# timgluz/teeline

Hardware: AMD Instinct MI355X
Metric: 2-opt candidate swaps evaluated/sec + final tour cost, TSPLIB EUC_2D n=10000 (higher is better)
Workload: dtype f32

## Files before the change

teeline_amd/csrc/two_opt_ref.hip:

```cpp
#include "tl_kernels.h"
#include "two_opt_common.h"

#include <type_traits>

#pragma clang fp contract(off)

namespace tl {

namespace {

constexpr uint32_t kNoKey = 0xFFFFFFFFu;
#if defined(TL_PROFILE2) || defined(TL_PROFILE3)
constexpr bool kProbeOwnsStats = true;
#else
constexpr bool kProbeOwnsStats = false;
#endif
#ifndef TL_RMAX
#define TL_RMAX 63
#endif
#ifndef TL_DENSE_ROWS
#define TL_DENSE_ROWS 8.0f
#endif
constexpr int kRMax = TL_RMAX;
constexpr uint32_t kQCap = 32;
constexpr uint32_t kPendMax = 64;
constexpr int kFlushSlots = 15;
constexpr int kFlushSlotsFx = 20;
constexpr int kMaxGroups = 4;


struct Ctl {
    uint2 kr[4];
    uint32_t desc[4];
    unsigned long long cnt[6];
    unsigned long long clk0, rt0;
    uint32_t bad_init;
    uint32_t nlong;
    uint32_t late_cur;
    uint32_t pad_[1];
    uint32_t pend[64];
};
constexpr size_t kCtlBytes = 384;
static_assert(sizeof(Ctl) <= kCtlBytes, "Ctl block");

constexpr size_t kXyBytes = 8, kFxLoBytes = 4, kFxHiBytes = 1, kPermBytes = 2, kNlPosBytes = 2;
constexpr size_t kTboxBytes = kMaxGroups * 64 * 16, kTmsqBytes = kMaxGroups * 64 * 4, kQueuesBytes = 32 * kQCap * 4;
constexpr size_t kNlLongBytes = (size_t)kNlLongCap * 16, kNlSurvBytes = 16 * 64 * 2;
static_assert(kQueuesBytes >= TL_TWO_OPT_NT * 4, "the hit lists double as the cost-sum scratch");

template <int CTRL>
__device__ __forceinline__ uint32_t dpp_shr0(uint32_t v)
{
    return (uint32_t)__builtin_amdgcn_update_dpp(0, (int)v, CTRL, 0xf, 0xf, true);
}
__device__ __forceinline__ uint32_t readlane_u(uint32_t v, uint32_t l) { return (uint32_t)__builtin_amdgcn_readlane((int)v, (int)l); }

template <int NT, int SLOTS, typename PT>
__device__ __forceinline__ uint32_t flush_deferred(const PT &P, uint16_t *perm, uint32_t g, uint32_t lo, uint32_t k, int lane, int wave)
{
    using Raw = decltype(pt_raw(P, 0u));
    const bool have = (uint32_t)lane < k;
    const uint32_t ghi = readlane_u(g, k - 1u);
    const uint32_t wfirst = lo + ((uint32_t)wave << 6);
    Raw val[SLOTS];
    uint32_t pk[SLOTS];
    if (wfirst <= ghi) {
        uint32_t gprev = dpp_shr0<0x111>(g);
        gprev = lane == 16 ? readlane_u(g, 15) : gprev;
        gprev = lane == 32 ? readlane_u(g, 31) : gprev;
        gprev = lane == 48 ? readlane_u(g, 47) : gprev;
        gprev = lane == 0 ? lo - 1u : gprev;
        const uint32_t start = gprev + 1u;
        const uint32_t len = have ? g - gprev : 0u;
        uint32_t pre = len;
        pre += dpp_shr0<0x112>(pre);
        pre += dpp_shr0<0x114>(pre);
        pre += dpp_shr0<0x118>(pre);
        if (k > 16u) {
            const uint32_t e0 = readlane_u(pre, 14), o0 = readlane_u(pre, 15);
            const uint32_t e1 = e0 + readlane_u(pre, 30), o1 = o0 + readlane_u(pre, 31);
            const uint32_t e2 = e1 + readlane_u(pre, 46), o2 = o1 + readlane_u(pre, 47);
            const bool odd = (lane & 1) != 0;
            uint32_t off = 0u;
            off = lane >= 16 ? (odd ? o0 : e0) : off;
            off = lane >= 32 ? (odd ? o1 : e1) : off;
            off = lane >= 48 ? (odd ? o2 : e2) : off;
            pre += off;
        }
        const uint32_t t_rev = readlane_u(pre, k - 1u);
        const bool isrev = ((k - 1u - (uint32_t)lane) & 1u) == 0u;
        const uint32_t base = lo + (isrev ? t_rev - pre : t_rev + pre - len);
        const uint32_t cst = isrev ? base + g : base - start;
#pragma unroll
        for (int q = 0; q < SLOTS; ++q) {
            const uint32_t w0 = wfirst + (uint32_t)(q * NT);
            if (w0 > ghi) break;
            const uint32_t p = w0 + (uint32_t)lane;
            const uint32_t w1 = (w0 + 63u < ghi) ? w0 + 63u : ghi;
            uint32_t m = (uint32_t)__builtin_popcountll(__builtin_amdgcn_ballot_w64(g < w0));
            const uint32_t mhi = (uint32_t)__builtin_popcountll(__builtin_amdgcn_ballot_w64(g < w1));
            const uint32_t c0 = readlane_u(cst, m);
            uint32_t dst = ((k - 1u - m) & 1u) == 0u ? c0 - p : c0 + p;
            for (++m; m <= mhi; ++m) {
                const uint32_t sm = readlane_u(start, m), cm = readlane_u(cst, m);
                const bool rv = ((k - 1u - m) & 1u) == 0u;
                dst = p >= sm ? (rv ? cm - p : cm + p) : dst;
            }
            if (p <= ghi) {
                val[q] = pt_raw(P, p);
                pk[q] = (uint32_t)perm[p] | (dst << 16);
            }
        }
    }
    TL_SYNC();
    if (wfirst <= ghi) {
#pragma unroll
        for (int q = 0; q < SLOTS; ++q) {
            const uint32_t w0 = wfirst + (uint32_t)(q * NT);
            if (w0 > ghi) break;
            if (w0 + (uint32_t)lane <= ghi) {
                const uint32_t dst = pk[q] >> 16;
                pt_put(P, dst, val[q]);
                perm[dst] = (uint16_t)pk[q];
            }
        }
    }
    TL_SYNC();
    return have ? g - (lo - 1u) : 0u;
}

template <int NT, typename PT>
__device__ __forceinline__ void reverse_segment(const PT &P, uint16_t *perm, uint32_t lo, uint32_t hi, int tid, uint16_t *pos = nullptr)
{
    const uint32_t half = (hi - lo + 1u) >> 1;
    for (uint32_t t = (uint32_t)tid; t < half; t += 2 * NT) {
        const uint32_t t2 = t + NT;
        const bool two = t2 < half;
        const auto x = pt_raw(P, lo + t), y = pt_raw(P, hi - t);
        const uint16_t u = perm[lo + t], v = perm[hi - t];
        uint16_t u2 = u, v2 = v;
        auto x2 = x, y2 = y;
        if (two) {
            x2 = pt_raw(P, lo + t2);
            y2 = pt_raw(P, hi - t2);
            u2 = perm[lo + t2];
            v2 = perm[hi - t2];
        }
        pt_put(P, lo + t, y);
        pt_put(P, hi - t, x);
        perm[lo + t] = v;
        perm[hi - t] = u;
        if (pos) {
            pos[v] = (uint16_t)(lo + t);
            pos[u] = (uint16_t)(hi - t);
        }
        if (two) {
            pt_put(P, lo + t2, y2);
            pt_put(P, hi - t2, x2);
            perm[lo + t2] = v2;
            perm[hi - t2] = u2;
            if (pos) {
                pos[v2] = (uint16_t)(lo + t2);
                pos[u2] = (uint16_t)(hi - t2);
            }
        }
    }
}

struct Cursor {
    uint32_t i0, j0;
    uint32_t np;
    uint32_t slot, par;
    uint32_t dirty_lo, dirty_hi;
    bool pruned;
};
struct Acct {
    uint64_t moves, reversed, rev_lane;
    float gap_est, since;
    bool improved;
    uint32_t *log;
    uint32_t log_cap, log_n;
};

__device__ __forceinline__ uint32_t block_rows(const Cursor &c, uint32_t nrows)
{
    return c.pruned ? ((uint32_t)kRMax < nrows - c.i0 ? (uint32_t)kRMax : nrows - c.i0) : 1u;
}

__device__ __forceinline__ void log_word(Acct &a, int lane, uint32_t w)
{
    if (a.log) {
        if (lane == 0 && a.log_n < a.log_cap) a.log[a.log_n] = w;
        a.log_n += 1u;
    }
}

template <bool CONTROL, int NT, int SLOTS, typename PT>
__device__ __forceinline__ void flush_pending(Cursor &c, Acct &a, const PT &P, uint16_t *perm, Ctl *ctl, int lane, int wave, bool sync_first)
{
    if (sync_first) TL_SYNC();
    uint32_t g = ctl->pend[lane];
    g = (uint32_t)lane < c.np ? g : 0xFFFFFFFFu;
    const uint32_t ghi = readlane_u(g, c.np - 1u);
    const uint32_t r = flush_deferred<NT, SLOTS>(P, perm, g, c.i0 + 1u, c.np, lane, wave);
    if (CONTROL) {
        a.rev_lane += r;
        if (a.log) {
            const uint32_t at = a.log_n + (uint32_t)lane;
            if ((uint32_t)lane < c.np && at < a.log_cap) a.log[at] = (c.i0 << 16) | g;
            a.log_n += c.np;
        }
    }
    const uint32_t t0 = c.i0 >> 6, t1 = ghi >> 6;
    c.dirty_lo = t0 < c.dirty_lo ? t0 : c.dirty_lo;
    c.dirty_hi = t1 > c.dirty_hi ? t1 : c.dirty_hi;
    c.np = 0;
}

template <bool CONTROL, int NT, int SLOTS, bool FOLD, typename PT>
__device__ __forceinline__ bool step_boundary(Cursor &c, Acct &a, const PT &P, uint16_t *perm, Ctl *ctl, const uint32_t *queues, uint32_t n, uint32_t nrows,
                                              uint32_t R, int lane, int wave, int tid, uint32_t my_hits, float &bx, float &by, bool &reload, float *tmsq)
{
    const uint2 kr = ctl->kr[c.slot];
    const uint32_t key = (uint32_t)__builtin_amdgcn_readfirstlane((int)kr.x);
    const uint32_t req = (uint32_t)__builtin_amdgcn_readfirstlane((int)kr.y);
    const float rowlen = (float)(n - 2u - c.i0);
    reload = false;
    if (!c.pruned) {
        bool flush = false, sync_first = false, next_row = false;
        if (key == kNoKey) {
            if (CONTROL) a.since += rowlen;
            flush = c.np != 0u;
            next_row = true;
        } else {
            const uint4 hv = *reinterpret_cast<const uint4 *>(queues + ((key & 0xFFFFu) * 2u + c.par) * kQCap);
            const uint32_t nh = (uint32_t)__builtin_amdgcn_readfirstlane((int)hv.x);
            const uint32_t resume = (uint32_t)__builtin_amdgcn_readfirstlane((int)hv.y);
            if (!CONTROL && (key & 0xFFFFu) == (uint32_t)wave && (uint32_t)lane < nh) ctl->pend[c.np + (uint32_t)lane] = my_hits;
            if (CONTROL) {
                a.moves += nh;
                a.since += (float)((key >> 16) - c.j0);
                a.gap_est = 0.5f * (a.gap_est + a.since);
                a.since = 0.0f;
                if (nh > 1u) a.gap_est = fminf(a.gap_est, 0.5f * a.gap_est + 16.0f);
                a.improved = true;
            }
            c.np += nh;
            c.j0 = resume;
            next_row = c.j0 > n - 2u;
            flush = next_row || c.np + kMaxChainHits > kPendMax;
            sync_first = true;
            if (!flush) {
                bx = __builtin_bit_cast(float, __builtin_amdgcn_readfirstlane((int)hv.z));
                by = __builtin_bit_cast(float, __builtin_amdgcn_readfirstlane((int)hv.w));
            }
        }
        if (flush) flush_pending<CONTROL, NT, SLOTS>(c, a, P, perm, ctl, lane, wave, sync_first);
        if (next_row) {
            c.i0 += 1u;
            c.j0 = c.i0 + 2u;
        }
        reload = flush || next_row;
    } else if (key == kNoKey) {
        if (CONTROL) a.since += (float)R * rowlen;
        c.i0 += R;
        c.j0 = c.i0 + 2u;
    } else {
        const uint32_t is = key >> 16, js = key & 0xFFFFu;
        const uint32_t t0 = is >> 6, t1 = js >> 6;
        const bool fold = FOLD && t0 == t1;
        if (fold && tid == 0) {
            const float m = fmaxf(sqdist(pt_get(P, is), pt_get(P, js)), sqdist(pt_get(P, is + 1u), pt_get(P, js + 1u)));
            if (m > tmsq[t0]) tmsq[t0] = m;
        }
        reverse_segment<NT>(P, perm, is + 1u, js, tid);
        TL_SYNC();
        if (CONTROL) {
            log_word(a, lane, key);
            a.since += (float)(is - c.i0) * rowlen;
            a.moves += 1u;
            a.reversed += (uint64_t)(js - is);
            a.since += (req != 0u && is > c.i0) ? (float)(js - (is + 2u)) : (float)(js - c.j0);
            a.gap_est = 0.5f * (a.gap_est + a.since);
            a.since = 0.0f;
            a.improved = true;
        }
        if (!fold) {
            c.dirty_lo = t0 < c.dirty_lo ? t0 : c.dirty_lo;
            c.dirty_hi = t1 > c.dirty_hi ? t1 : c.dirty_hi;
        }
        c.i0 = is;
        c.j0 = js + 1u;
        if (c.j0 > n - 2u) {
            c.i0 += 1u;
            c.j0 = c.i0 + 2u;
        }
    }
    c.slot = c.slot == 2u ? 0u : c.slot + 1u;
    c.par ^= 1u;
    return c.i0 >= nrows || req != 0u;
}


struct NlLds {
    uint16_t *pos;
    uint4 *longe;
    uint16_t *surv;
};

template <typename PT>
__device__ __forceinline__ uint32_t nl_r2_bits(const PT &P, uint32_t k, uint32_t n)
{
    const float2 pk = pt_get(P, k);
    uint32_t r2 = 0u;
    if (k >= 1u) r2 = __builtin_bit_cast(uint32_t, sqdist(pt_get(P, k - 1u), pk));
    if (k + 1u < n) {
        const uint32_t s = __builtin_bit_cast(uint32_t, sqdist(pk, pt_get(P, k + 1u)));
        r2 = s > r2 ? s : r2;
// ... 225 lines not shown
                        if (q + 1u < (uint32_t)kLateRowsPerWave) recw = load_rec(cida, cidb, r + 1u);
                        else recw = load_rec(ida, idb, r0n);
                    }
                    const float rax = readlane_f(rp.x, r), ray = readlane_f(rp.y, r);
                    const float rbx = readlane_f(rq.x, r), rby = readlane_f(rq.y, r);
                    const float rsqab = readlane_f(rowsq, r);
                    const uint32_t jmin = (i == i0) ? j0 : (i + 2u);
                    tc.prow += 1u;
                    uint32_t col = 0xFFFFFFFFu;
                    bool listed = false;
                    if (nl_rows) {
                        const uint32_t w = cur & 0xFFFFu;
                        const bool bad = lane == 0 ? !((__builtin_bit_cast(uint32_t, rsqab) >> 16) < w) : (lane == 2 && w != 0u);
                        if (!__builtin_amdgcn_ballot_w64(bad)) {
                            listed = true;
                            uint32_t u = lane >= kNlSurv0 ? surv8 : w;
                            const bool valid = lane >= kNlRecA0 && u != 0xFFFFu;
                            u = valid ? u : 0u;
                            const uint32_t pu = L.pos[u];
                            uint32_t j = lane < kNlRecB0 ? pu : pu - 1u;
                            j = valid ? j : 0xFFFFFFFFu;
                            col = nl_pass(P, n, j, jmin, rax, ray, rbx, rby, rsqab, lane, tc);
                            if (ns > (uint32_t)kNlSurvSlots) {
                                const uint32_t q2 = (uint32_t)kNlSurvSlots + (uint32_t)lane;
                                const bool v2 = q2 < ns;
                                const uint32_t u2 = v2 ? sv[q2 < 64u ? q2 : 0u] : 0u;
                                const uint32_t p2 = L.pos[u2];
                                const uint32_t c2 = nl_pass(P, n, v2 ? p2 - 1u : 0xFFFFFFFFu, jmin, rax, ray, rbx, rby, rsqab, lane, tc);
                                col = c2 < col ? c2 : col;
                            }
                        }
                    }
                    if (!listed) {
                        float4 box[kMaxGroups];
                        float msq[kMaxGroups];
#pragma unroll
                        for (int gI = 0; gI < kMaxGroups; ++gI) {
                            if (gI < G) {
                                box[gI] = tbox[((uint32_t)gI << 6) + (uint32_t)lane];
                                msq[gI] = tmsq[((uint32_t)gI << 6) + (uint32_t)lane];
                            }
                        }
                        col = row_tiles<true>(P, n, G, box, msq, jmin, rax, ray, rbx, rby, rsqab, lane, tc);
                    }
                    TL_LSTAMP(2);
#ifdef TL_PROFILE_LATE
                    lq[3] += 1;
#endif
                    if (col == 0xFFFFFFFFu) continue;
                    if (lane == 0) lds_min_u32_fenced(keyslot, (i << 16) | col);
                    stop = true;
                    break;
                }
                g = gn;
            }
            TL_LSTAMP(5);
        }
#ifdef TL_PROFILE_LATE
        const uint64_t tb2 = __builtin_amdgcn_s_memtime();
#endif
        TL_SYNC();
#ifdef TL_PROFILE_LATE
        lq[4] += __builtin_amdgcn_s_memtime() - tb2;
#endif
        const uint32_t key = (uint32_t)__builtin_amdgcn_readfirstlane((int)ctl->kr[slot].x);
        if (key == kNoKey) {
            i0 += R;
            j0 = i0 + 2u;
        } else {
            const uint32_t is = key >> 16, js = key & 0xFFFFu;
            const uint32_t t0 = is >> 6, t1 = js >> 6;
            if (t0 == t1 && tid == 0) {
                const float m = fmaxf(sqdist(pt_get(P, is), pt_get(P, js)), sqdist(pt_get(P, is + 1u), pt_get(P, js + 1u)));
                if (m > tmsq[t0]) tmsq[t0] = m;
            }
            reverse_segment<NT>(P, perm, is + 1u, js, tid, L.pos);
            TL_SYNC();
            if (control) {
                log_word(acct, lane, key);
                acct.moves += 1u;
                acct.reversed += (uint64_t)(js - is);
            }
            improved = true;
            if (t0 != t1) {
                dirty_lo = t0 < dirty_lo ? t0 : dirty_lo;
                dirty_hi = t1 > dirty_hi ? t1 : dirty_hi;
            }
            fix = true;
            fi = is;
            fj = js;
            i0 = is;
            j0 = js + 1u;
            if (j0 > n - 2u) {
                i0 += 1u;
                j0 = i0 + 2u;
            }
        }
        slot = slot_next;
    }
#ifdef TL_PROFILE_LATE
    if (d == 0 && lane == 0 && (wave == 1 || wave == 9))
        printf("late phase, wave %d: chunk set-up %lu, prefilter %lu, rows %lu cycles in %lu rows (%lu per row), B2 wait %lu, other %lu\n", wave, lq[0], lq[1], lq[2], lq[3],
               lq[2] / (lq[3] ? lq[3] : 1), lq[4], lq[5]);
#endif
    (void)d;
}

}

template <int NT, bool PRUNE, bool COUNT, bool FX, bool NL = false>
__global__ __launch_bounds__(NT, 4) void k_two_opt_ref_lds(TwoOptBatchArgs A)
{
    static_assert(!NL || (PRUNE && !FX), "late phase: the float2 forms with pruning");
    constexpr int kSlots = FX ? kFlushSlotsFx : kFlushSlots;
    extern __shared__ __attribute__((aligned(16))) unsigned char smem[];
    constexpr int NW = NT / 64;
    static_assert(NW == 16 || NW == 8 || NW == 4, "16 waves; 8 or 4 for two or four descents per CU");
    const uint32_t n = A.n, npad = A.n_pad;
    const uint32_t ntile = npad >> 6;
    const int G = (int)((ntile + 63u) >> 6);
    using PT = typename std::conditional<FX, PtsFx, float2 *>::type;
    PT P;
    uint16_t *perm;
    unsigned char *tailp;
    if constexpr (FX) {
        P.lo = reinterpret_cast<uint32_t *>(smem);
        P.hi = reinterpret_cast<uint8_t *>(smem + (size_t)npad * kFxLoBytes);
        P.inv = A.fx_inv;
        perm = reinterpret_cast<uint16_t *>(smem + (size_t)npad * (kFxLoBytes + kFxHiBytes));
        tailp = smem + (size_t)npad * (kFxLoBytes + kFxHiBytes + kPermBytes);
    } else {
        P = reinterpret_cast<float2 *>(smem);
        perm = reinterpret_cast<uint16_t *>(smem + (size_t)npad * kXyBytes);
        tailp = smem + (size_t)npad * (kXyBytes + kPermBytes);
    }
    float4 *tbox = reinterpret_cast<float4 *>(tailp);
    float *tmsq = reinterpret_cast<float *>(tailp + kTboxBytes);
    Ctl *ctl = reinterpret_cast<Ctl *>(tailp + kTboxBytes + kTmsqBytes);
    uint32_t *queues = reinterpret_cast<uint32_t *>(reinterpret_cast<unsigned char *>(ctl) + kCtlBytes);
    float *scratch = reinterpret_cast<float *>(queues);
    NlLds L{nullptr, nullptr, nullptr};
    if constexpr (NL) {
        unsigned char *nlp = reinterpret_cast<unsigned char *>(queues) + kQueuesBytes;
        L.pos = reinterpret_cast<uint16_t *>(nlp);
        L.longe = reinterpret_cast<uint4 *>(nlp + (size_t)npad * kNlPosBytes);
        L.surv = reinterpret_cast<uint16_t *>(nlp + (size_t)npad * kNlPosBytes + kNlLongBytes);
    }

    const int tid = threadIdx.x, lane = tid & 63;
    const int wave = __builtin_amdgcn_readfirstlane(tid >> 6);
    const uint32_t d = blockIdx.x;
    const float2 *__restrict__ xy = A.xy;

    if (A.init_mode == TL_INIT_ARRAY) {
        const uint32_t *__restrict__ src = A.init + (size_t)d * n;
        if (tid == 0) ctl->bad_init = 0u;
        TL_SYNC();
        bool bad = false;
        for (uint32_t k = tid; k < n; k += NT) {
            const uint32_t v = src[k];
            bad |= v >= n;
            perm[k] = (uint16_t)v;
        }
        if (bad) ctl->bad_init = 1u;
        TL_SYNC();
        if (ctl->bad_init) {
            if (tid == 0) {
                A.out_cost[d] = __builtin_nanf("");
                uint64_t *st = A.out_stats + (size_t)d * TL_STATS_STRIDE;
                for (int q = 0; q < TL_STATS_STRIDE; ++q) st[q] = 0;
                st[3] = 2;
            }
            return;
        }
    } else {
        for (uint32_t k = tid; k < n; k += NT) perm[k] = (uint16_t)k;
    }
    if (A.init_mode == TL_INIT_SEEDED) {
        uint16_t *draws = reinterpret_cast<uint16_t *>(smem);
        const uint64_t s = A.seed + (uint64_t)(A.first + d);
        for (uint32_t i = 1 + tid; i < n; i += NT) {
            const uint64_t kth = (uint64_t)(n - 1 - i);
            draws[i] = (uint16_t)(splitmix64_at(s, kth) % ((uint64_t)i + 1));
        }
        TL_SYNC();
        if (tid == 0) {
            for (uint32_t i = n - 1; i >= 1; --i) {
                const uint32_t j = draws[i];
                const uint16_t t = perm[i];
                perm[i] = perm[j];
                perm[j] = t;
            }
        }
    }
    if (tid < 4) ctl->kr[tid] = make_uint2(kNoKey, 0u);
    if (tid < 6) ctl->cnt[tid] = 0ull;
    if (tid == 0) {
        ctl->nlong = 0u;
        ctl->clk0 = __builtin_amdgcn_s_memtime();
        ctl->rt0 = __builtin_amdgcn_s_memrealtime();
    }
    for (uint32_t k = tid; k < (uint32_t)kMaxGroups * 64u; k += NT) {
        const float inf = __builtin_inff();
        tbox[k] = make_float4(inf, inf, -inf, -inf);
        tmsq[k] = -1.0f;
    }
    TL_SYNC();
    if constexpr (FX) {
        for (uint32_t k = tid; k < npad; k += NT) {
            const uint2 g = (k < n) ? A.fx_xy[perm[k]] : make_uint2(0u, 0u);
            pt_put(P, k, PtsFx::Raw{g.x, g.y});
        }
    } else {
        for (uint32_t k = tid; k < npad; k += NT) P[k] = (k < n) ? xy[perm[k]] : make_float2(0.f, 0.f);
    }
    TL_SYNC();
    for (uint32_t t = (uint32_t)wave; t < ntile; t += NW) build_tile_meta(P, n, t, lane, tbox, tmsq);
    TL_SYNC();

    const uint32_t nrows = n - 3;
    const uint32_t last_tile = n >= 2 ? (n - 2u) >> 6 : 0u;
    uint32_t sweeps = 1, step = 0, status = 0;
    uint64_t moves = 0, reversed = 0;
    uint64_t rev_lane = 0;
    typename std::conditional<COUNT, TileCounts, NoCounts>::type tc;

    enum : uint32_t { OP_GO = 0u, OP_LATE = 1u, OP_EXIT = 2u };
    bool go_late = false;
    uint32_t n_late_steps = 0;
    uint64_t late_clk = 0;
    constexpr int NWK = NW - 1;
    constexpr uint32_t kLead = kDenseLead < (uint32_t)NWK ? kDenseLead : (uint32_t)NWK;
    if (n >= 4 && wave == 0) {
        Cursor c{0u, 2u, 0u, 0u, 0u, 0xFFFFFFFFu, 0u, false};
        Acct acct{0ull, 0ull, 0ull, 0.0f, 0.0f, false, A.move_log ? A.move_log + (size_t)d * A.log_cap : nullptr, A.log_cap, 0u};
        bool need_desc = true;
        uint32_t n_desc = 0, n_pruned_steps = 0;
        uint64_t sweep_moves0 = 0;
#ifdef TL_PROFILE2
        uint64_t q2[13] = {0, 0, 0, 0, 0, 0, 0, 0, 0, 0, 0, 0, 0};
        uint64_t t_it = __builtin_amdgcn_s_memtime();
#endif
#ifdef TL_PROFILE4
        uint64_t q4[10] = {0, 0, 0, 0, 0, 0, 0, 0, 0, 0};
        uint64_t q4c[3] = {0, 0, 0}, t4b = __builtin_amdgcn_s_memtime();
        uint64_t q4m[3] = {0, 0, 0};
        uint64_t q4l[4] = {0, 0, 0, 0};
        uint64_t t4 = __builtin_amdgcn_s_memtime();
#endif
        for (;;) {
            if (need_desc) {
                ++n_desc;
                bool done = false, new_sweep = false;
                if (c.i0 >= nrows) {
                    if (!acct.improved) {
                        done = true;
                    } else if (sweeps >= A.max_sweeps) {
                        status = 1;
                        done = true;
                    } else if (NL && sweeps + 1u >= A.nl.sweep_min && acct.moves - sweep_moves0 < (uint64_t)A.nl.moves_max) {
                        go_late = true;
                    } else {
#ifdef TL_PROFILE4
                        if (d == 0 && lane == 0)
                            printf("sweep %u: dense hit in lead tiles %lu steps %lu cyc, behind %lu steps %lu cyc\n", sweeps, q4l[0], q4l[1], q4l[2], q4l[3]);
                        for (int q = 0; q < 4; ++q) q4l[q] = 0;
                        if (d == 0 && lane == 0)
                            printf("sweep %u: dense hit %lu steps %lu cyc | dense none %lu steps %lu cyc, tiles %lu of which with valid boxes %lu | pruned hit %lu steps %lu cyc | pruned none %lu steps %lu cyc\n",
                                   sweeps, q4[0], q4[1], q4[2], q4[3], q4[8], q4[9], q4[4], q4[5], q4[6], q4[7]);
                        for (int q = 0; q < 10; ++q) q4[q] = 0;
#endif
                        acct.improved = false;
                        ++sweeps;
                        sweep_moves0 = acct.moves;
                        c.i0 = 0;
                        c.j0 = 2;
                        if (NL) {
                            c.dirty_lo = 0u;
                            c.dirty_hi = ntile - 1u;
                            new_sweep = true;
                        }
                        log_word(acct, lane, 0xFFFFFFFFu);
                    }
                }
                c.pruned = PRUNE && !done && fmaxf(acct.gap_est, acct.since) > TL_DENSE_ROWS * (float)(n - 2u - c.i0);
                if (lane == 0) {
                    *reinterpret_cast<uint2 *>(ctl->desc) = make_uint2((done ? OP_EXIT : go_late ? OP_LATE : OP_GO) | (c.pruned ? 4u : 0u) | (new_sweep ? 8u : 0u), c.i0 | (c.j0 << 16));
                    if (NL) ctl->desc[2] = sweeps;
                }
                TL_SYNC();
                if (lane == 0) {
                    ctl->kr[0].y = 0u;
                    ctl->kr[1].y = 0u;
                    ctl->kr[2].y = 0u;
                }
                if (c.np) flush_pending<true, NT, kSlots>(c, acct, P, perm, ctl, lane, wave, false);
                if (done || go_late) break;
            }
            const uint32_t slot_next = c.slot == 2u ? 0u : c.slot + 1u;
            if (lane == 0) ctl->kr[slot_next].x = kNoKey;
            ++step;
            n_pruned_steps += c.pruned ? 1u : 0u;
            const uint32_t R = block_rows(c, nrows);
            if (c.pruned) {
                if (c.dirty_lo <= c.dirty_hi) {
#ifdef TL_PROFILE4
                    const uint64_t tm0 = __builtin_amdgcn_s_memtime();
                    q4m[2] += c.dirty_hi - c.dirty_lo + 1u;
#endif
                    for (uint32_t t = c.dirty_lo; t <= c.dirty_hi; t += (uint32_t)NW) build_tile_meta(P, n, t, lane, tbox, tmsq);
                    c.dirty_lo = 0xFFFFFFFFu;
                    c.dirty_hi = 0;
                    TL_SYNC();
#ifdef TL_PROFILE4
                    q4m[0] += __builtin_amdgcn_s_memtime() - tm0;
                    q4m[1] += 1;
#endif
                }
            } else {
#ifdef TL_PROFILE4
                const uint64_t tb0 = __builtin_amdgcn_s_memtime();
#endif
                TL_SYNC();
#ifdef TL_PROFILE4
                {
                    const uint64_t tb1 = __builtin_amdgcn_s_memtime();
                    q4c[0] += tb0 - t4b;
                    q4c[1] += tb1 - tb0;
                    q4c[2] += 1;
                }
#endif
            }
            TL_SYNC();
#ifdef TL_PROFILE4
            t4b = __builtin_amdgcn_s_memtime();
#endif
#ifdef TL_PROFILE2
            const bool was_pruned = c.pruned;
            const uint64_t moves_before = acct.moves;
#endif
#ifdef TL_PROFILE4
            const bool was_pruned4 = c.pruned;
            const uint64_t moves_before4 = acct.moves;
            const uint32_t t0_4 = c.j0 >> 6, dlo4 = c.dirty_lo, dhi4 = c.dirty_hi;
            const uint32_t key4 = (uint32_t)__builtin_amdgcn_readfirstlane((int)ctl->kr[c.slot].x);
#endif
            float bx_ = 0.f, by_ = 0.f;
// ... 151 lines not shown
                        box[gI] = tbox[((uint32_t)gI << 6) + (uint32_t)lane];
                        msq[gI] = tmsq[((uint32_t)gI << 6) + (uint32_t)lane];
                    }
                }
                for (int r = wk; r < (int)R; r += NWK) {
                    const uint32_t i = i0 + (uint32_t)r;
#ifdef TL_PROFILE4
                    qp[1] += 1;
#endif
                    if (r >= NWK) {
                        const uint32_t kb = (uint32_t)__builtin_amdgcn_readfirstlane((int)*keyslot);
                        if (kb != kNoKey && (kb >> 16) < i) break;
                    }
                    const float rax = readlane_f(rp.x, r), ray = readlane_f(rp.y, r);
                    const float rbx = readlane_f(rp.x, r + 1), rby = readlane_f(rp.y, r + 1);
                    const float rsqab = readlane_f(rowsq, r);
                    const uint32_t jmin = (r == 0) ? j0 : (i + 2u);
                    const uint32_t tmin = jmin >> 6;
                    uint64_t hm = 0;
                    uint32_t t = 0;
                    tc.prow += 1u;
#pragma unroll
                    for (int gI = 0; gI < kMaxGroups; ++gI) {
                        if (gI < G && (((uint32_t)gI + 1u) << 6) > tmin) {
                            const uint32_t tl = ((uint32_t)gI << 6) + (uint32_t)lane;
                            uint64_t m = __builtin_amdgcn_ballot_w64(tl >= tmin) &
                                         (__builtin_amdgcn_ballot_w64(box_lb(rax, ray, box[gI]) < rsqab) | __builtin_amdgcn_ballot_w64(box_lb(rbx, rby, box[gI]) < msq[gI]));
                            tc.l0 += 64u;
                            while (m != 0) {
                                t = ((uint32_t)gI << 6) + (uint32_t)(__builtin_ffsll((long long)m) - 1);
                                m &= m - 1;
                                tc.ptile += 1u;
#ifdef TL_PROFILE4
                                qp[2] += 1;
#endif
                                if constexpr (NL) {
                                    const uint32_t kb = (uint32_t)__builtin_amdgcn_readfirstlane((int)*keyslot);
                                    if (kb != kNoKey && (kb >> 16) < i) goto rows_done;
                                }
                                hm = tile_improving_mask<PRUNE>(P, n, t << 6, jmin, rax, ray, rbx, rby, rsqab, lane, tc);
                                if (hm) goto row_hit;
                            }
                        }
                    }
                    continue;
                row_hit:
                    if (lane == 0) lds_min_u32_fenced(keyslot, (i << 16) | ((t << 6) + (uint32_t)(__builtin_ffsll((long long)hm) - 1)));
                    break;
                }
            rows_done:;
#ifdef TL_PROFILE4
                qp[0] += __builtin_amdgcn_s_memtime() - tp0;
                qp[3] += 1;
#endif
            }
#ifdef TL_PROFILE4
            const uint64_t tpb = __builtin_amdgcn_s_memtime();
#endif
            TL_SYNC();
#ifdef TL_PROFILE4
            if (c.pruned) qp[4] += __builtin_amdgcn_s_memtime() - tpb;
#endif
            TL_STAMP3(4);
#ifdef TL_PROFILE3
            if (!c.pruned) {
                const uint32_t key3 = (uint32_t)__builtin_amdgcn_readfirstlane((int)ctl->kr[c.slot].x);
                const int ty = key3 == kNoKey ? 2 : (((key3 >> 16) >> 6) < (c.j0 >> 6) + kLead ? 0 : 1);
                for (int q = 0; q < 5; ++q) q3[ty][q] += d3[q];
                q3[ty][5] += 1;
            } else {
                t3 = __builtin_amdgcn_s_memtime();
            }
#endif
            need_desc = step_boundary<false, NT, kSlots, NL>(c, acct, P, perm, ctl, queues, n, nrows, R, lane, wave, tid, my_hits, bx, by, reload, tmsq);
        }
#ifdef TL_PROFILE4
        if (d == 0 && lane == 0 && (wave == 1 || wave == 8))
            printf("wave %d, pruned steps of the main loop: %lu; scan %lu cycles per step, %lu rows and %lu tile passes per step, B2 wait %lu\n", wave, qp[3], qp[0] / (qp[3] ? qp[3] : 1),
                   qp[1] * 100 / (qp[3] ? qp[3] : 1), qp[2] * 100 / (qp[3] ? qp[3] : 1), qp[4] / (qp[3] ? qp[3] : 1));
#endif
        if constexpr (NL) {
            if (go_late) late_phase<NT>(A, P, perm, tbox, tmsq, ctl, L, d, n, nrows, ntile, G, c.dirty_lo, c.dirty_hi, acct, sweeps, step, status, n_late_steps, tc, lane, wave, tid);
        }
#ifdef TL_PROFILE3
        if (d == 0 && lane == 0 && (wave == 1 || wave == 6))
            for (int ty = 0; ty < 3; ++ty)
                printf("wave %d, dense steps %s: %lu steps; per step: to the lead round %lu, lead tile %lu, B1 wait %lu, round 2 %lu, B2 wait %lu\n", wave,
                       ty == 0 ? "with the first hit in the lead tiles" : ty == 1 ? "with the first hit behind them" : "without a hit", q3[ty][5],
                       q3[ty][0] / (q3[ty][5] ? q3[ty][5] : 1), q3[ty][1] / (q3[ty][5] ? q3[ty][5] : 1), q3[ty][2] / (q3[ty][5] ? q3[ty][5] : 1),
                       q3[ty][3] / (q3[ty][5] ? q3[ty][5] : 1), q3[ty][4] / (q3[ty][5] ? q3[ty][5] : 1));
#endif
    }

    uint32_t *__restrict__ out = A.out_pos + (size_t)d * n;
    for (uint32_t k = tid; k < n; k += NT) out[k] = perm[k];

    if constexpr (COUNT) {
        if (lane == 0) {
            atomicAdd(&ctl->cnt[0], (unsigned long long)tc.l0);
            atomicAdd(&ctl->cnt[1], (unsigned long long)tc.l1);
            atomicAdd(&ctl->cnt[2], (unsigned long long)tc.l2);
            atomicAdd(&ctl->cnt[3], (unsigned long long)tc.l3);
            atomicAdd(&ctl->cnt[4], (unsigned long long)tc.prow);
            atomicAdd(&ctl->cnt[5], (unsigned long long)tc.ptile);
        }
    }
    float total = 0.0f;
    if (n >= 2) total = dist(pt_get(P, n - 1), pt_get(P, 0));
    TL_SYNC();
    for (uint32_t base = 0; base + 1 < n; base += NT) {
        const uint32_t k = base + tid;
        scratch[tid] = (k + 1 < n) ? dist(pt_get(P, k), pt_get(P, k + 1)) : 0.0f;
        TL_SYNC();
        if (tid == 0) {
            const uint32_t cnt = (n - 1 - base) < (uint32_t)NT ? (n - 1 - base) : (uint32_t)NT;
            const float4 *s4 = reinterpret_cast<const float4 *>(scratch);
            uint32_t qd = 0;
            for (; qd + 4 <= cnt; qd += 4) {
                const float4 v = s4[qd >> 2];
                total += v.x;
                total += v.y;
                total += v.z;
                total += v.w;
            }
            for (; qd < cnt; ++qd) total += scratch[qd];
        }
        TL_SYNC();
    }
    if (wave == 0) {
#pragma unroll
        for (int sft = 32; sft >= 1; sft >>= 1) {
            const uint32_t lo32 = (uint32_t)__shfl_xor((int)(uint32_t)rev_lane, sft), hi32 = (uint32_t)__shfl_xor((int)(uint32_t)(rev_lane >> 32), sft);
            rev_lane += ((uint64_t)hi32 << 32) | lo32;
        }
        reversed += rev_lane;
    }
    if (tid == 0) {
        A.out_cost[d] = total;
        uint64_t *st = A.out_stats + (size_t)d * TL_STATS_STRIDE;
        st[0] = sweeps;
        st[1] = moves;
        st[2] = reversed;
        st[3] = status;
        st[4] = step;
        if constexpr (!kProbeOwnsStats) {
        st[5] = ctl->cnt[0];
        st[6] = ctl->cnt[1];
        st[7] = ctl->cnt[2];
        st[8] = ctl->cnt[3];
        st[11] = ctl->cnt[4];
        st[12] = ctl->cnt[5];
        st[9] = __builtin_amdgcn_s_memtime() - ctl->clk0;
        st[10] = __builtin_amdgcn_s_memrealtime() - ctl->rt0;
        }
    }
}

static size_t lds_bytes(uint32_t n, size_t per_city, uint32_t *n_pad_out)
{
    const uint32_t n_pad = ((n + 64u + 63u) / 64u) * 64u;
    if (n_pad_out) *n_pad_out = n_pad;
    if (n_pad > (uint32_t)kMaxGroups * 64u * 64u) return ~(size_t)0;
    return (size_t)n_pad * per_city + kTboxBytes + kTmsqBytes + kCtlBytes + kQueuesBytes;
}

size_t two_opt_ref_lds_bytes(uint32_t n, uint32_t *n_pad_out) { return lds_bytes(n, kXyBytes + kPermBytes, n_pad_out); }

size_t two_opt_ref_fx_lds_bytes(uint32_t n) { return lds_bytes(n, kFxLoBytes + kFxHiBytes + kPermBytes, nullptr); }

bool two_opt_ref_fx_pays(uint32_t n, uint32_t count, int cus, int lds_budget)
{
    const size_t plain = two_opt_ref_lds_bytes(n, nullptr), fx = two_opt_ref_fx_lds_bytes(n);
    if (cus <= 0 || count <= (uint32_t)cus) return false;
    const bool two = 2 * plain > (size_t)lds_budget && 2 * fx <= (size_t)lds_budget && (size_t)n <= (size_t)kFlushSlotsFx * 512;
    const bool four = count > 2u * (uint32_t)cus && 4 * plain > (size_t)lds_budget && 4 * fx <= (size_t)lds_budget &&
                      (size_t)n <= (size_t)kFlushSlotsFx * 256;
    return two || four;
}

__global__ __launch_bounds__(256) void k_fx_encode(const float2 *__restrict__ xy, uint32_t n, double scale, double inv, uint2 *__restrict__ out,
                                                   uint32_t *__restrict__ bad)
{
    const uint32_t c = blockIdx.x * 256u + threadIdx.x;
    if (c >= n) return;
    const float2 p = xy[c];
    const double gx = rint((double)p.x * scale), gy = rint((double)p.y * scale);
    bool ok = gx >= 0.0 && gy >= 0.0 && gx < 1048576.0 && gy < 1048576.0;
    uint2 g = make_uint2(0u, 0u);
    if (ok) {
        const uint32_t kx = (uint32_t)gx, ky = (uint32_t)gy;
        g = make_uint2(kx | ((ky & 0xFFFu) << 20), ky >> 12);
        const float2 q = fx_decode(g.x, g.y, inv);
        ok = __float_as_uint(q.x) == __float_as_uint(p.x) && __float_as_uint(q.y) == __float_as_uint(p.y);
    }
    out[c] = g;
    if (!ok) atomicAdd(bad, 1u);
}

hipError_t launch_fx_encode(const float2 *xy, uint32_t n, double scale, uint2 *out, uint32_t *bad, hipStream_t s)
{
    hipLaunchKernelGGL(k_fx_encode, dim3((n + 255u) / 256u), dim3(256), 0, s, xy, n, scale, 1.0 / scale, out, bad);
    return hipGetLastError();
}

template <int NT, bool PRUNE, bool COUNT, bool FX, bool NL = false>
static hipError_t launch_one(const TwoOptBatchArgs &A, uint32_t count, size_t lds, hipStream_t s)
{
    auto kern = k_two_opt_ref_lds<NT, PRUNE, COUNT, FX, NL>;
    hipError_t e = allow_max_lds(reinterpret_cast<const void *>(kern));
    if (e != hipSuccess) return e;
    hipLaunchKernelGGL(kern, dim3(count), dim3(NT), lds, s, A);
    return hipGetLastError();
}

template <int NT, bool FX>
static hipError_t launch_nt(const TwoOptBatchArgs &B, uint32_t count, size_t lds, bool prune, bool count_work, hipStream_t s)
{
    if constexpr (NT == 1024 && !FX) {
        if (prune && B.nl.rec)
            return count_work ? launch_one<NT, true, true, FX, true>(B, count, lds, s) : launch_one<NT, true, false, FX, true>(B, count, lds, s);
    }
    if constexpr ((NT == 512 || NT == 256) && !FX) {
        if (prune && B.nl.rec) return launch_one<NT, true, false, FX, true>(B, count, lds, s);
    }
    if constexpr (NT == TL_TWO_OPT_NT && !FX) {
        if (count_work) return prune ? launch_one<NT, true, true, FX>(B, count, lds, s) : launch_one<NT, false, true, FX>(B, count, lds, s);
    }
    return prune ? launch_one<NT, true, false, FX>(B, count, lds, s) : launch_one<NT, false, false, FX>(B, count, lds, s);
}

hipError_t launch_two_opt_ref_lds(const TwoOptBatchArgs &A, uint32_t count, bool prune, hipStream_t s, bool count_work, int cus, int lds_budget,
                                  int force_nt)
{
    uint32_t n_pad = 0;
    const size_t lds = two_opt_ref_lds_bytes(A.n, &n_pad);
    TwoOptBatchArgs B = A;
    B.n_pad = n_pad;
    if (A.fx_xy && A.fx_inv != 0.0) {
        const size_t fl = two_opt_ref_fx_lds_bytes(A.n);
        if (cus > 0 && count > 2u * (uint32_t)cus && 4 * fl <= (size_t)lds_budget && (size_t)A.n <= (size_t)kFlushSlotsFx * 256)
            return launch_nt<256, true>(B, count, fl, prune, count_work, s);
        if ((size_t)A.n > (size_t)kFlushSlotsFx * 512) return hipErrorInvalidValue;
        return launch_nt<512, true>(B, count, fl, prune, count_work, s);
    }
    const int nt = two_opt_ref_pick_nt(A.n, count, cus, lds_budget, force_nt);
    const size_t nl_lds = two_opt_ref_nl_lds_bytes(A.n);
    const bool nl = prune && B.nl.rec && two_opt_ref_nl_form(A.n, count, cus, lds_budget, force_nt);
    if (!nl) B.nl.rec = nullptr;
    if (nt == 256) return launch_nt<256, false>(B, count, nl ? nl_lds : lds, prune, count_work, s);
    if (nt == 512) return launch_nt<512, false>(B, count, nl ? nl_lds : lds, prune, count_work, s);
    return launch_nt<TL_TWO_OPT_NT, false>(B, count, nl ? nl_lds : lds, prune, count_work, s);
}

int two_opt_ref_pick_nt(uint32_t n, uint32_t count, int cus, int lds_budget, int force_nt)
{
    const size_t lds = two_opt_ref_lds_bytes(n, nullptr);
    const size_t fit = lds ? (size_t)lds_budget / lds : 1;
    int nt = TL_TWO_OPT_NT;
    if (force_nt) {
        nt = force_nt;
    } else if (cus > 0 && count > (uint32_t)cus) {
        if (fit >= 4 && count > 2u * (uint32_t)cus) nt = 256;
        else if (fit >= 2) nt = 512;
    }
    while (nt < TL_TWO_OPT_NT && (size_t)n > (size_t)kFlushSlots * (size_t)nt) nt *= 2;
    return nt;
}

bool two_opt_ref_nl_form(uint32_t n, uint32_t count, int cus, int lds_budget, int force_nt)
{
    if (TL_TWO_OPT_NT != 1024 || n <= (uint32_t)kNlKB + 1u || n > 65535u) return false;
    const size_t nl_lds = two_opt_ref_nl_lds_bytes(n);
    if (nl_lds > (size_t)lds_budget) return false;
    const int nt = two_opt_ref_pick_nt(n, count, cus, lds_budget, force_nt);
    if (nt == 1024) return true;
    if (nt == 512) return force_nt == 512 || 2 * nl_lds <= (size_t)lds_budget;
    if (nt == 256) return force_nt == 256 || 4 * nl_lds <= (size_t)lds_budget;
    return false;
}

size_t two_opt_ref_nl_lds_bytes(uint32_t n)
{
    uint32_t n_pad = 0;
    const size_t base = two_opt_ref_lds_bytes(n, &n_pad);
    if (base == ~(size_t)0) return base;
    return base + (size_t)n_pad * kNlPosBytes + kNlLongBytes + kNlSurvBytes;
}

bool two_opt_ref_nl_applies(uint32_t n, uint32_t count, int cus, int lds_budget, int force_nt)
{
    return two_opt_ref_nl_form(n, count, cus, lds_budget, force_nt);
}

}
```

Baseline: 1631 billion.

## Parallelize seeded Fisher-Yates shuffle via counting-sort chain resolution

```diff
diff --git a/teeline_amd/csrc/two_opt_ref.hip b/teeline_amd/csrc/two_opt_ref.hip
--- a/teeline_amd/csrc/two_opt_ref.hip
+++ b/teeline_amd/csrc/two_opt_ref.hip
@@ -20,6 +20,15 @@
 #endif
 #ifndef TL_DENSE_ROWS
 #define TL_DENSE_ROWS 8.0f
+#endif
+#ifdef TL_PROFILE_PROLOGUE
+#define TL_PROLOGUE_STAMP(var, sync) \
+    if (sync) TL_SYNC();             \
+    const uint64_t var = __builtin_amdgcn_s_memtime()
+#else
+#define TL_PROLOGUE_STAMP(var, sync) \
+    do {                             \
+    } while (0)
 #endif
 constexpr int kRMax = TL_RMAX;
 constexpr uint32_t kQCap = 32;
@@ -164,6 +173,72 @@
                 pos[u2] = (uint16_t)(hi - t2);
             }
         }
+    }
+}
+
+template <int NT>
+__device__ __forceinline__ void seeded_start_tour(unsigned char *pts, uint16_t *perm, uint32_t n, uint32_t npad, uint64_t s, int tid)
+{
+    uint16_t *draws = reinterpret_cast<uint16_t *>(pts);
+    uint32_t *offw = reinterpret_cast<uint32_t *>(pts + (size_t)npad * 2);
+    uint16_t *ent = reinterpret_cast<uint16_t *>(pts + (size_t)npad * 4);
+    uint32_t *wtot = reinterpret_cast<uint32_t *>(pts + (size_t)npad * 6);
+    const int lane = tid & 63;
+    for (uint32_t w = tid; w < (npad >> 1); w += NT) offw[w] = 0u;
+    TL_SYNC();
+    for (uint32_t i = 1 + tid; i < n; i += NT) {
+        const uint64_t kth = (uint64_t)(n - 1 - i);
+        const uint32_t p = (uint32_t)(splitmix64_at(s, kth) % ((uint64_t)i + 1));
+        draws[i] = (uint16_t)p;
+        atomicAdd(&offw[p >> 1], 1u << ((p & 1u) << 4));
+    }
+    TL_SYNC();
+    const uint32_t wpt = ((npad >> 1) + (uint32_t)NT - 1u) / (uint32_t)NT;
+    const uint32_t w0 = (uint32_t)tid * wpt;
+    const uint32_t w1 = w0 + wpt < (npad >> 1) ? w0 + wpt : (npad >> 1);
+    uint32_t sum = 0u;
+    for (uint32_t w = w0; w < w1; ++w) {
+        const uint32_t v = offw[w];
+        sum += (v & 0xFFFFu) + (v >> 16);
+    }
+    uint32_t incl = sum;
+#pragma unroll
+    for (int sft = 1; sft < 64; sft <<= 1) {
+        const uint32_t up = (uint32_t)__shfl_up((int)incl, sft);
+        incl += lane >= sft ? up : 0u;
+    }
+    if (lane == 63) wtot[tid >> 6] = incl;
+    TL_SYNC();
+    uint32_t run = incl - sum;
+    for (int q = 0; q < (tid >> 6); ++q) run += wtot[q];
+    for (uint32_t w = w0; w < w1; ++w) {
+        const uint32_t v = offw[w];
+        const uint32_t a = run, b = run + (v & 0xFFFFu);
+        run = b + (v >> 16);
+        offw[w] = a | (b << 16);
+    }
+    TL_SYNC();
+    for (uint32_t i = 1 + tid; i < n; i += NT) {
+        const uint32_t p = draws[i], sh = (p & 1u) << 4;
+        const uint32_t old = atomicAdd(&offw[p >> 1], 1u << sh);
+        ent[(old >> sh) & 0xFFFFu] = (uint16_t)i;
+    }
+    TL_SYNC();
+    for (uint32_t i = tid; i < n; i += NT) {
+        uint32_t p = i ? (uint32_t)draws[i] : 0u, cur = i;
+        for (;;) {
+            const uint32_t hi = (offw[p >> 1] >> ((p & 1u) << 4)) & 0xFFFFu;
+            const uint32_t lo = p ? (offw[(p - 1u) >> 1] >> (((p - 1u) & 1u) << 4)) & 0xFFFFu : 0u;
+            uint32_t best = 0xFFFFFFFFu;
+            for (uint32_t k = lo; k < hi; ++k) {
+                const uint32_t t = ent[k];
+                best = (t > cur && t < best) ? t : best;
+            }
+            if (best == 0xFFFFFFFFu) break;
+            p = best;
+            cur = best;
+        }
+        perm[i] = (uint16_t)p;
     }
 }
 
@@ -695,6 +770,12 @@
     const uint32_t d = blockIdx.x;
     const float2 *__restrict__ xy = A.xy;
 
+#ifdef TL_SHUFFLE_SERIAL
+    constexpr bool kSeededByGroup = false;
+#else
+    constexpr bool kSeededByGroup = !FX;
+#endif
+    TL_PROLOGUE_STAMP(t_pro0, false);
     if (A.init_mode == TL_INIT_ARRAY) {
         const uint32_t *__restrict__ src = A.init + (size_t)d * n;
         if (tid == 0) ctl->bad_init = 0u;
@@ -716,10 +797,13 @@
             }
             return;
         }
+    } else if (kSeededByGroup && A.init_mode == TL_INIT_SEEDED) {
+        seeded_start_tour<NT>(smem, perm, n, npad, A.seed + (uint64_t)(A.first + d), tid);
     } else {
         for (uint32_t k = tid; k < n; k += NT) perm[k] = (uint16_t)k;
     }
-    if (A.init_mode == TL_INIT_SEEDED) {
+    TL_PROLOGUE_STAMP(t_pro1, true);
+    if (!kSeededByGroup && A.init_mode == TL_INIT_SEEDED) {
         uint16_t *draws = reinterpret_cast<uint16_t *>(smem);
         const uint64_t s = A.seed + (uint64_t)(A.first + d);
         for (uint32_t i = 1 + tid; i < n; i += NT) {
@@ -736,6 +820,7 @@
             }
         }
     }
+    TL_PROLOGUE_STAMP(t_pro2, true);
     if (tid < 4) ctl->kr[tid] = make_uint2(kNoKey, 0u);
     if (tid < 6) ctl->cnt[tid] = 0ull;
     if (tid == 0) {
@@ -1193,6 +1278,10 @@
         st[12] = ctl->cnt[5];
         st[9] = __builtin_amdgcn_s_memtime() - ctl->clk0;
         st[10] = __builtin_amdgcn_s_memrealtime() - ctl->rt0;
+#ifdef TL_PROFILE_PROLOGUE
+        st[11] = ctl->clk0 - t_pro0;
+        st[12] = t_pro2 - t_pro1;
+#endif
         }
     }
 }
```

Measured after the change: 1644 billion, median of 6. About the same (+0.8%).
